# baresip/re

Hardware: AMD Instinct MI355X
Metric: GiB/s + Mpkt/s SRTP protect+unprotect, 1200B RTP pkts, device-resident (higher is better)
Workload: dtype u8

## Files before the change

re_amd/csrc/hip/k_ctr_fused.h:

```cpp
#pragma once
#include "k_ctr_fast.h"
#include "plan_common.h"

struct FArgs {
	KArgs a;
	struct sgpu_fused p;
};

#define FZ_BLOCK CTRF_BLOCK

struct FShared {
	uint32_t t;
	uint32_t fail;
	uint32_t hl0, ssrc0, seq0;
	uint32_t excl;
	uint32_t xfail;
	uint32_t wsum[FZ_BLOCK / 64];
	uint32_t seq[FZ_BLOCK + 2];
};

#ifdef FZ_WTIME
#define FZ_WTIME_MAX 4096u
#define FZ_WREC 24u
__device__ uint64_t g_fzw[FZ_WREC * FZ_WTIME_MAX];
#define FZ_STAMP(k)                                                          \
	do {                                                                 \
		if (threadIdx.x == 0 && S.t < FZ_WTIME_MAX)                  \
			g_fzw[FZ_WREC * S.t + 18u + (k)] =                   \
				__builtin_amdgcn_s_memrealtime();            \
	} while (0)
#else
#define FZ_STAMP(k) do { } while (0)
#endif

template <bool PROT>
__device__ __forceinline__ int fz_plan(const FArgs &fa, FShared &S,
				       uint8_t *smem, FastPkt &fp)
{
	const KArgs &a = fa.a;
	const struct sgpu_fused &P = fa.p;
	const struct sgpu_plan_in &in = P.in;
	const uint32_t tid = threadIdx.x, B = FZ_BLOCK;
	const uint32_t lane = tid & 63u, wv = tid >> 6;
	const uint64_t asz = a.asz;
	const uint32_t n = in.n;

	if (tid == 0) {
		S.t = atomicAdd(P.ticket, 1u) - P.tbase;
		S.fail = 0;
	}
	__syncthreads();
	FZ_STAMP(0);
	const uint32_t t = S.t;
	const uint32_t base = t * B, i = base + tid;
	const bool live = i < n;
	uint32_t p = 0, e = 0, cp = 0;
	struct sgpu_hdr h;
	h.ssrc = 0; h.seq = 0; h.err_pos = 0; h.hdr_len = 0xffffffffu;
	if (live) {
		p = P.pos[i];
		e = P.end[i];
		cp = P.cap ? P.cap[i] : 0u;
		const uint32_t left = (e > p && e <= asz) ? e - p : 0u;
		h = parse_rtp_hdr(a.arena + p, p, left);
	}
	if (tid < 3) {
		if (tid == 0) {
			const uint32_t q = P.pos[0], qe = P.end[0];
			const uint32_t left = (qe > q && qe <= asz) ? qe - q : 0u;
			const struct sgpu_hdr h0 = parse_rtp_hdr(a.arena + q, q,
								 left);
			S.hl0 = h0.hdr_len;
			S.ssrc0 = h0.ssrc;
			S.seq0 = h0.seq;
			if (t == 0) {
				P.out_next->fail = 0;
				P.out_next->nfail = 0;
				if (P.cm_out)
					*P.cm_out = P.comp;
			}
		}
		else if (base >= tid) {
			const uint32_t q = P.pos[base - tid];
			uint32_t sv = 0;
			if ((uint64_t)q + 4u <= asz)
				sv = (uint32_t)a.arena[q + 2] << 8 | a.arena[q + 3];
			S.seq[2 - tid] = sv;
		}
	}
#ifndef FZ_FILL_LOOP
	static_assert(FZ_BLOCK == 1024, "tt4_fill_b1024");
	tt4_fill_b1024(smem, a.t0);
#else
	tt4_fill(smem, a.t0);
#endif
	FZ_STAMP(4);
	if (live) {
		P.hdr[i] = h;
		P.es[i] = e;
		S.seq[tid + 2] = h.seq;
	}
	__syncthreads();
	FZ_STAMP(1);

	const uint32_t hl0 = S.hl0;
	const uint32_t ssrc0 = in.ssrc_any ? S.ssrc0 : in.ssrc;
	const uint32_t s_l0 = in.fresh ? S.seq0 : in.s_l;
	const uint32_t seq = h.seq;
	uint32_t f = 0, sb = 0;
	bool wrap = false;
	if (live) {
		sb = i == 0 ? s_l0 : S.seq[tid + 1];
		const uint32_t L = e - p;
		f |= plan_header_flags(h.hdr_len, hl0, h.ssrc, ssrc0,
				       PLAN_SSRC_PARSED, L, in.tag, 1, PROT);
		f |= plan_window_flags(p, e, P.cap != NULL, cp, asz, in.maxlen,
				       in.need, PROT);
		const struct plan_ord o = plan_order(seq, sb, i + 1 >= n, PROT);
		f |= o.flags;
		wrap = o.wrap;
		if (i == 0) {
			P.out->ssrc0 = h.ssrc;
			P.out->hl0 = h.hdr_len;
		}
	}
	if (tid == 0 && in.pred && *in.pred)
		f |= SPF_PRED;
	if (f)
		atomicOr(&S.fail, f);
	const uint64_t m = __ballot(wrap);
	if (lane == 0)
		S.wsum[wv] = (uint32_t)__popcll(m);
	__syncthreads();
	FZ_STAMP(2);

	if (wv == 0) {
		const uint32_t tot = wave_sum(lane < B / 64u ? S.wsum[lane] : 0u);
		const struct fz_prefix pf = fz_lookback(P.agg, P.epoch, t, lane,
							S.fail, tot,
							&P.out->fail);
		if (lane == 0) {
			S.excl = pf.excl;
			S.xfail = pf.fail;
		}
	}
	__syncthreads();
	FZ_STAMP(3);
	if (!live)
		return -1;
	if (S.xfail) {
		P.desc[i] = 0;
		return -1;
	}

	uint32_t pre = (uint32_t)__popcll(m & ((1ull << lane) - 1ull));
	for (uint32_t q = 0; q < wv; q++)
		pre += S.wsum[q];
	const uint32_t roc = in.roc + S.excl + pre + (wrap ? 1u : 0u);
	const struct plan_idx x = plan_index(roc, wrap, sb, seq, PROT);
	const uint64_t ix = x.ix;
	if (!PROT) {
		bool ok;
		if (i == 0) {
			ok = plan_new_first(ix, in.lix, in.bitmap);
		}
		else {
			const uint32_t psb = i == 1 ? s_l0 : S.seq[tid];
			ok = plan_new_later(ix, plan_prev_index(roc, wrap, psb, sb),
					    in.lix);
		}
		if (!ok)
			atomicOr(&P.out->fail, (uint32_t)SPF_REPLAY);
	}
	P.desc[i] = d_desc(ix, x.fl);
	const uint32_t t0 = n > SGPU_PLAN_TAIL ? n - SGPU_PLAN_TAIL : 0u;
	if (i >= t0)
		P.out->tail_ix[i - t0] = ix;
	if (i + 1 == n) {
		P.out->s_l_last = plan_s_l_after(seq, sb, wrap);
		P.out->wraps = roc - in.roc;
	}
	P.end[i] = e + (uint32_t)P.delta;
	P.err[i] = 0;
	fp.p = i;
	fp.off = p;
	fp.L = e - p;
	fp.hl = h.hdr_len;
	fp.ssrc = h.ssrc;
	fp.ixhi = (uint32_t)(ix >> 16);
	fp.ixlo = (uint32_t)(ix & 0xffffu);
	fp.roc = roc;
	return (int)((hl0 >> 2) & 3u);
}

template <int NR, bool PROT>
__global__ void
__attribute__((amdgpu_flat_work_group_size(1, FZ_BLOCK)))
__attribute__((amdgpu_waves_per_eu(FZ_BLOCK / 256, 8)))
k_ctr_fused(const FArgs fa)
{
#ifdef FZ_WTIME
	uint64_t t_start = 0;
	if (threadIdx.x == 0)
		t_start = __builtin_amdgcn_s_memrealtime();
#endif
	__shared__ __attribute__((aligned(16))) uint8_t smem[TT4_BYTES];
	__shared__ FShared S;
	FastPkt f;
	const int cls = fz_plan<PROT>(fa, S, smem, f);
#ifdef FZ_WTIME
	if (threadIdx.x == 0 && S.t < FZ_WTIME_MAX) {
		uint32_t hw;
		asm volatile("s_getreg_b32 %0, hwreg(HW_REG_HW_ID)" : "=s"(hw));
		g_fzw[FZ_WREC * S.t] = t_start;
		g_fzw[FZ_WREC * S.t + 1u] = hw;
	}
#endif
	if (cls < 0)
		return;
	const uint32_t ci = fa.p.comp;
	switch (cls) {
	case 0: ctr_fast_pkt<NR, 0, PROT>(fa.a, smem, f, ci); break;
	case 1: ctr_fast_pkt<NR, 1, PROT>(fa.a, smem, f, ci); break;
	case 2: ctr_fast_pkt<NR, 2, PROT>(fa.a, smem, f, ci); break;
	case 3: ctr_fast_pkt<NR, 3, PROT>(fa.a, smem, f, ci); break;
	default: break;
	}
#ifdef FZ_WTIME
	if ((threadIdx.x & 63u) == 0) {
		const uint32_t t = S.t;
		if (t < FZ_WTIME_MAX)
			g_fzw[FZ_WREC * t + 2u + threadIdx.x / 64u] =
				__builtin_amdgcn_s_memrealtime();
	}
#endif
}

#ifndef LP_PPT
#define LP_PPT 4
#endif
#define LP_WG (FZ_BLOCK * LP_PPT)

struct LpShared {
	uint32_t t, fail, hl0, ssrc0, seq0, excl, xfail;
	uint32_t wsum[LP_PPT][FZ_BLOCK / 64];
	uint32_t seq[LP_WG + 2];
};

template <bool PROT>
__global__ void __launch_bounds__(FZ_BLOCK)
k_lp_plan(const FArgs fa)
{
	__shared__ LpShared S;
	const KArgs &a = fa.a;
	const struct sgpu_fused &P = fa.p;
	const struct sgpu_plan_in &in = P.in;
	const uint32_t tid = threadIdx.x;
	const uint32_t lane = tid & 63u, wv = tid >> 6;
	const uint64_t asz = a.asz;
	const uint32_t n = in.n;

	if (tid == 0) {
		S.t = atomicAdd(P.ticket, 1u) - P.tbase;
		S.fail = 0;
	}
	__syncthreads();
	const uint32_t t = S.t;
	const uint32_t base = t * LP_WG;
	uint32_t pv[LP_PPT], ev[LP_PPT], cv[LP_PPT], w0[LP_PPT], w2[LP_PPT];
#pragma unroll
	for (int j = 0; j < LP_PPT; j++) {
		const uint32_t i = base + j * FZ_BLOCK + tid;
		pv[j] = ev[j] = cv[j] = 0;
		if (i < n) {
			pv[j] = P.pos[i];
			ev[j] = P.end[i];
			cv[j] = P.cap ? P.cap[i] : 0u;
		}
	}
#pragma unroll
	for (int j = 0; j < LP_PPT; j++) {
		const uint32_t p = pv[j], e = ev[j];
		w0[j] = w2[j] = 0;
		if (base + j * FZ_BLOCK + tid < n && e > p && e <= asz &&
		    e - p >= 12 && !(p & 3u)) {
			w0[j] = *(const uint32_t *)(a.arena + p);
			w2[j] = *(const uint32_t *)(a.arena + p + 8);
		}
	}
	if (tid < 3) {
		if (tid == 0) {
			const uint32_t q = P.pos[0], qe = P.end[0];
			const uint32_t left = (qe > q && qe <= asz) ? qe - q : 0u;
			const struct sgpu_hdr h0 = parse_rtp_hdr(a.arena + q, q,
								 left);
			S.hl0 = h0.hdr_len;
			S.ssrc0 = h0.ssrc;
			S.seq0 = h0.seq;
			if (t == 0) {
				P.out_next->fail = 0;
				P.out_next->nfail = 0;
				if (P.cm_out)
					*P.cm_out = P.comp;
				for (uint32_t c = 0; c < 4; c++)
					P.out->skip[c] =
						h0.hdr_len == 0xffffffffu ||
						((h0.hdr_len >> 2) & 3u) != c;
			}
		}
		else if (base >= tid) {
			const uint32_t q = P.pos[base - tid];
			uint32_t sv = 0;
			if ((uint64_t)q + 4u <= asz)
				sv = (uint32_t)a.arena[q + 2] << 8 | a.arena[q + 3];
			S.seq[2 - tid] = sv;
		}
	}
	struct sgpu_hdr hv[LP_PPT];
// ... 215 lines not shown
```

re_amd/csrc/hip/srtp_kernels.hip:

```cpp
#include <hip/hip_runtime.h>
#include <stddef.h>
#include <errno.h>
#include <stdio.h>
#include <string.h>
#include "../srtpgpu.h"
#include "kern_common.h"
#include "plan_common.h"
#include "k_ctr_fused.h"

#ifndef EAUTH
#define EAUTH 217
#endif


__device__ uint32_t g_T0[256];
__device__ uint8_t g_sbox[256];


__device__ uint8_t d_xt(uint8_t a) { return (uint8_t)((a << 1) ^ ((a & 0x80) ? 0x1b : 0)); }

__device__ void d_aes_expand(const uint8_t *key, uint32_t nk, uint8_t *rkb)
{
	uint32_t nr = nk + 6, i;
	uint8_t rcon = 1;
// ... 489 lines not shown
{
	const uint32_t left = (e > p && e <= asz) ? e - p : 0u;
	if (left < 12u + tag)
		return 0;
	const uint8_t *q = arena + e - 4u - tag;
	return (uint32_t)q[0] << 24 | (uint32_t)q[1] << 16 |
	       (uint32_t)q[2] << 8 | q[3];
}

__global__ void __launch_bounds__(PLAN_BLOCK)
k_rp_plan(const uint8_t *__restrict__ arena, uint64_t asz,
	  const struct sgpu_rfused R)
{
	__shared__ uint32_t ssrc0s, vw[PLAN_BLOCK + 1];
	const struct sgpu_rplan_in &in = R.in;
	const uint32_t tid = threadIdx.x;
	const uint32_t i = blockIdx.x * PLAN_BLOCK + tid;
	if (tid == 0) {
		const uint32_t q = R.pos[0], qe = R.end[0];
		const uint32_t left = (qe > q && qe <= asz) ? qe - q : 0u;
		ssrc0s = left >= 8 ? (uint32_t)arena[q + 4] << 24 |
				     (uint32_t)arena[q + 5] << 16 |
				     (uint32_t)arena[q + 6] << 8 | arena[q + 7]
				   : 0u;
		if (blockIdx.x == 0) {
			R.out_next->fail = 0;
			R.out_next->nfail = 0;
			if (R.cm_out)
				*R.cm_out = R.comp;
		}
		vw[0] = (!in.prot && i > 0 && i - 1 < in.n) ?
			rp_word(arena, asz, R.pos[i - 1], R.end[i - 1], in.tag)
			: 0u;
	}
	const bool live = i < in.n;
	uint32_t p = 0, e = 0, c = 0, v = 0;
	struct sgpu_hdr h;
	h.ssrc = 0; h.seq = 0; h.err_pos = 0; h.hdr_len = 0xffffffffu;
	if (live) {
		p = R.pos[i];
		e = R.end[i];
		c = R.cap ? R.cap[i] : 0u;
		const uint32_t left = (e > p && e <= asz) ? e - p : 0u;
		if (left >= 8) {
			const uint8_t *b = arena + p;
			h.ssrc = (uint32_t)b[4] << 24 | (uint32_t)b[5] << 16 |
				 (uint32_t)b[6] << 8 | b[7];
			h.hdr_len = 8;
		}
		if (!in.prot)
			v = rp_word(arena, asz, p, e, in.tag);
		R.hdr[i] = h;
		R.es[i] = e;
	}
	vw[tid + 1] = v;
	__syncthreads();
	if (!live)
		return;
	const uint32_t ssrc0 = in.ssrc_any ? ssrc0s : in.ssrc;
	const struct plan_rtcp r = plan_rtcp_packet(
		in, i, h.hdr_len != 0xffffffffu, h.ssrc, ssrc0, e - p,
		plan_window_flags(p, e, R.cap != NULL, c, asz, in.maxlen, in.need,
				  in.prot),
		v, vw[tid]);
	rplan_emit(r, i, in.n, h.ssrc, R.desc, R.out);
}


static char g_err[256];
static int g_inited;
static struct sgpu_session *g_table;
static struct sgpu_sstate *g_sst;
static uint32_t g_table_cap;
static struct sgpu_keyreq *g_req_dev;

extern "C" struct sgpu_sstate *sgpu_sst_table(void)
{
	return g_sst;
}
static uint32_t *g_slot_dev;
static uint32_t g_req_cap;

static const uint32_t *g_T0_dev;

static int herr(hipError_t e, const char *what)
{
	if (e == hipSuccess)
		return 0;
	snprintf(g_err, sizeof(g_err), "%s: %s", what, hipGetErrorString(e));
	return EIO;
}

extern "C" const char *sgpu_last_error(void) { return g_err; }

static uint8_t h_xt(uint8_t a) { return (uint8_t)((a << 1) ^ ((a & 0x80) ? 0x1b : 0)); }

extern "C" int sgpu_init(void)
{
	int n = 0;
	if (g_inited)
		return 0;
	if (hipGetDeviceCount(&n) != hipSuccess || n <= 0) {
		snprintf(g_err, sizeof(g_err), "no HIP device visible");
		return ENODEV;
	}
	uint8_t sbox[256];
	uint32_t T0[256];
	for (int x = 0; x < 256; x++) {
		uint8_t inv = 0;
		for (int y = 1; x && y < 256; y++) {
			uint8_t a = (uint8_t)x, b = (uint8_t)y, r = 0;
			while (b) {
				if (b & 1)
					r ^= a;
				a = h_xt(a);
				b >>= 1;
			}
			if (r == 1) {
				inv = (uint8_t)y;
				break;
			}
		}
		uint8_t s = inv;
		s = (uint8_t)(inv ^ (uint8_t)((inv << 1) | (inv >> 7)) ^
			      (uint8_t)((inv << 2) | (inv >> 6)) ^
			      (uint8_t)((inv << 3) | (inv >> 5)) ^
			      (uint8_t)((inv << 4) | (inv >> 4)) ^ 0x63);
		sbox[x] = s;
	}
	for (int x = 0; x < 256; x++) {
		uint8_t s = sbox[x], s2 = h_xt(s), s3 = (uint8_t)(s2 ^ s);
		T0[x] = (uint32_t)s2 | (uint32_t)s << 8 | (uint32_t)s << 16 |
			(uint32_t)s3 << 24;
	}
	int e = herr(hipMemcpyToSymbol(HIP_SYMBOL(g_sbox), sbox, 256), "sbox");
	if (!e)
		e = herr(hipMemcpyToSymbol(HIP_SYMBOL(g_T0), T0, 1024), "T0");
	if (!e)
		e = herr(hipGetSymbolAddress((void **)&g_T0_dev, HIP_SYMBOL(g_T0)),
			 "T0 address");
	if (e)
		return e;
	g_inited = 1;
	return 0;
}

extern "C" int sgpu_table_reserve(uint32_t nsessions)
{
	if (nsessions <= g_table_cap)
		return 0;
	uint32_t cap = g_table_cap ? g_table_cap : 1024;
	while (cap < nsessions)
		cap *= 2;
	struct sgpu_session *nt = NULL;
	struct sgpu_sstate *ns = NULL;
	int e = herr(hipMalloc(&nt, (size_t)cap * sizeof(*nt)), "table alloc");
	if (!e)
		e = herr(hipMalloc(&ns, (size_t)cap * sizeof(*ns)),
			 "state table alloc");
	if (e) {
		(void)hipFree(nt);
		return e;
	}
	if (g_table) {
		e = herr(hipMemcpy(nt, g_table,
				   (size_t)g_table_cap * sizeof(*nt),
				   hipMemcpyDeviceToDevice), "table grow");
		if (!e)
			e = herr(hipMemcpy(ns, g_sst,
					   (size_t)g_table_cap * sizeof(*ns),
					   hipMemcpyDeviceToDevice),
				 "state table grow");
		(void)hipDeviceSynchronize();
		(void)hipFree(g_table);
		(void)hipFree(g_sst);
	}
	g_table = nt;
	g_sst = ns;
	g_table_cap = cap;
	return e;
}


__global__ void k_gate_pred(const uint32_t *pred, uint32_t *fail)
{
	if (*pred)
		atomicOr(fail, (uint32_t)SPF_PRED);
}

__global__ void k_gate_set(const uint32_t *fail, const uint32_t *nfail,
			   uint32_t *gate)
{
	*gate = (*fail || (nfail && *nfail)) ? 1u : 0u;
}

extern "C" int sgpu_gate_pred(const uint32_t *pred, uint32_t *fail,
			      void *stream)
{
	hipLaunchKernelGGL(k_gate_pred, dim3(1), dim3(1), 0,
			   (hipStream_t)stream, pred, fail);
	return herr(hipGetLastError(), "k_gate_pred launch");
}

extern "C" int sgpu_gate_set(const uint32_t *fail, const uint32_t *nfail,
			     uint32_t *gate, void *stream)
{
	hipLaunchKernelGGL(k_gate_set, dim3(1), dim3(1), 0,
			   (hipStream_t)stream, fail, nfail, gate);
	return herr(hipGetLastError(), "k_gate_set launch");
}


__global__ void k_sst_zero(const uint32_t *slot, uint32_t n,
			   struct sgpu_sstate *sst)
{
	const uint32_t i = blockIdx.x * blockDim.x + threadIdx.x;
	if (i < n)
		sst[slot[i]] = sgpu_sstate{};
}

static_assert(sizeof(struct sgpu_sstate) == 32 &&
	      offsetof(struct sgpu_sstate, flags) == 12,
	      "sst_ld/sst_st move the state as two 16-byte words");

__device__ __forceinline__ void sst_ld(const struct sgpu_sstate *p, uint4 &a,
// ... 526 lines not shown
			      (hipStream_t)stream, sgpu_ctr_fast_mk_block(),
			      "k_ctr_fast_mk", nr, prot, 4);
		if (!e && !prot && c->flist) {
			const uint32_t g = c->n < 1024u ? c->n : 1024u;
			hipLaunchKernelGGL(nr == 10 ? sgpu_pick_ctr10_fast(0, 3)
						    : sgpu_pick_ctr14_fast(0, 3),
					   dim3(g), dim3(256), 0,
					   (hipStream_t)stream, a);
			e = herr(hipGetLastError(), "refix mk launch");
		}
		return e;
	}
	kfn_t f = mode == SGPU_MODE_GCM ?
			  sgpu_pick_gcm(true, c->uniform != 0, nr, prot)
		  : nr == 10 ? sgpu_pick_ctr10(true, c->uniform != 0, shift, prot)
			     : sgpu_pick_ctr14(true, c->uniform != 0, shift, prot);
	if (!f) {
		snprintf(g_err, sizeof(g_err), "no kernel for mode %d nr %d",
			 mode, nr);
		return EINVAL;
	}
	KArgs a;
	memset(&a, 0, sizeof(a));
	a.arena = arena;
	a.asz = arena_size;
	a.comps = (const struct sgpu_comp *)g_table;
	a.t0 = g_T0_dev;
	a.verdict = c->verdict;
	a.save = c->save;
	a.c = *c;
	return launch(f, a, c->n,
		      c->undo ? -1 : prof_slot(mode, nr, shift < 0 ? 3 : shift,
					       prot),
		      (hipStream_t)stream,
		      mode == SGPU_MODE_GCM ? sgpu_gcm_block(c->uniform != 0)
					    : sgpu_ctr_block(c->uniform != 0, prot),
		      mode == SGPU_MODE_GCM ?
			      (c->uniform ? "k_gcmu" : "k_gcm_compact") :
		      shift < 0 ? (c->uniform ? "k_ctr_hmac_any_uni"
					      : "k_ctr_hmac_any") :
				  (c->uniform ? "k_ctr_hmac_uni"
					      : "k_ctr_hmac_compact"),
		      nr, prot, mode == SGPU_MODE_CTR && shift < 0 ? 4 : 1);
}


static void fz_args(FArgs &fa, uint8_t *arena, uint64_t asz,
		   const struct sgpu_fused *f)
{
	memset(&fa, 0, sizeof(fa));
	KArgs &a = fa.a;
	a.arena = arena;
	a.asz = asz;
	a.comps = (const struct sgpu_comp *)g_table;
	a.t0 = g_T0_dev;
	a.verdict = f->verdict;
	a.save = f->save;
	a.c.pos = f->pos;
	a.c.end = f->es;
	a.c.hdr = f->hdr;
	a.c.desc = f->desc;
	a.c.compmap = f->cm_out;
	a.c.n = f->in.n;
	a.c.verdict = f->verdict;
	a.c.save = f->save;
	a.c.nfail = &f->out->nfail;
	a.c.flist = f->flist;
	a.c.uniform = 2;
	fa.p = *f;
}

extern "C" unsigned sgpu_fused_block(void)
{
	return FZ_BLOCK;
}

extern "C" int sgpu_run_fused(uint8_t *arena, uint64_t arena_size,
			      struct sgpu_fused *f, int nr, void *stream)
{
	FArgs fa;
	if (!f->in.n || (nr != 10 && nr != 14))
		return EINVAL;
	const int prot = f->in.prot != 0;
	const uint32_t nwg = (f->in.n + FZ_BLOCK - 1) / FZ_BLOCK;
	f->ntickets = nwg;
	fz_args(fa, arena, arena_size, f);
	return launch_fused(sgpu_pick_fused(nr, prot, 0), fa, nwg * FZ_BLOCK,
			    f->in.n, prof_slot(SGPU_MODE_CTR, nr, 3, prot),
			    (hipStream_t)stream, FZ_BLOCK, "k_ctr_fused", nr,
			    prot, &f->prof_id);
}

extern "C" int sgpu_run_fzplan(uint8_t *arena, uint64_t arena_size,
			       struct sgpu_fused *f, void *stream)
{
	FArgs fa;
	if (!f->in.n)
		return EINVAL;
	const uint32_t wg = sgpu_lp_wg();
	const uint32_t nwg = (f->in.n + wg - 1) / wg;
	f->ntickets = nwg;
	f->prof_id = 0;
	fz_args(fa, arena, arena_size, f);
	hipLaunchKernelGGL(sgpu_pick_fzplan(f->in.prot != 0), dim3(nwg),
			   dim3(FZ_BLOCK), 0, (hipStream_t)stream, fa);
	return herr(hipGetLastError(), "plan launch");
}

extern "C" int sgpu_fused_undo(uint8_t *arena, uint64_t arena_size,
			       const struct sgpu_fused *f, int nr, int prot,
			       void *stream)
{
	FArgs fa;
	if (!f->in.n || (nr != 10 && nr != 14) || f->shift > 3)
		return EINVAL;
	fz_args(fa, arena, arena_size, f);
	hipLaunchKernelGGL(sgpu_pick_fused(nr, prot, 1),
			   dim3((f->in.n + FZ_BLOCK - 1) / FZ_BLOCK),
			   dim3(FZ_BLOCK), 0, (hipStream_t)stream, fa);
	return herr(hipGetLastError(), "fused undo launch");
}

extern "C" int sgpu_fused_refix(uint8_t *arena, uint64_t arena_size,
				const struct sgpu_fused *f, int nr,
				void *stream)
{
	FArgs fa;
	if (!f->in.n || (nr != 10 && nr != 14))
		return EINVAL;
	fz_args(fa, arena, arena_size, f);
	const uint32_t g = f->in.n < 1024u ? f->in.n : 1024u;
	hipLaunchKernelGGL(nr == 10 ? sgpu_pick_ctr10_fast(0, 2)
				    : sgpu_pick_ctr14_fast(0, 2),
			   dim3(g), dim3(256), 0, (hipStream_t)stream, fa.a);
	return herr(hipGetLastError(), "fused refix launch");
}

extern "C" int sgpu_parse_headers(const uint8_t *arena, uint64_t arena_size,
				  const uint32_t *pos, const uint32_t *end,
				  struct sgpu_hdr *out, uint32_t *eix, uint32_t n,
				  int rtcp, void *stream)
{
	if (!n)
		return 0;
	struct sgpu_prologue pro;
	memset(&pro, 0, sizeof(pro));
	return sgpu_parse_prologue(arena, arena_size, pos, end, out, eix, n,
				   rtcp, &pro, stream);
}

extern "C" int sgpu_parse_prologue(const uint8_t *arena, uint64_t arena_size,
				   const uint32_t *pos, const uint32_t *end,
				   struct sgpu_hdr *out, uint32_t *eix,
				   uint32_t n, int rtcp,
				   const struct sgpu_prologue *pro,
				   void *stream)
{
	if (!n)
		return 0;
	hipLaunchKernelGGL(k_parse, dim3((n + 255) / 256), dim3(256), 0,
			   (hipStream_t)stream, arena, arena_size, pos, end, out,
			   eix, n, rtcp, *pro);
	return herr(hipGetLastError(), "k_parse launch");
}

__global__ void k_rx_pack(const struct sgpu_hdr *__restrict__ hd,
			  const int32_t *__restrict__ res, uint32_t ssrc0,
			  uint32_t *__restrict__ out, uint32_t n)
// ... 604 lines not shown
```

re_amd/csrc/host/batch_dev.c:

```c
#include <errno.h>
#include <pthread.h>
#include <stdatomic.h>
#include <stdio.h>
#include <stdlib.h>
#include <string.h>
#include <time.h>
#include "re_mem.h"
#include "re_mbuf.h"
#include "re_srtp.h"
#include "re_srtp_batch.h"
#include "re_rtcp_batch.h"
#include "../srtpgpu.h"
#include "../hip/plan_rx_rule.h"
#include "bp_layout.h"
#include "fault.h"
#include "pool.h"
#include "srtp_int.h"


static struct sgpu_compact compact_of(const struct srtp_batch_dev *d,
				      const struct ws_layout *L)
{
	return (struct sgpu_compact){
		.pos = d->pos, .end = L->es, .hdr = L->hdr, .desc = L->desc,
// ... 269 lines not shown
}

static int plan_out_back(struct dcall *k, struct sgpu_plan_out *out,
			 void *host, void *stream)
{
	const int sync = k->sync;
	int err = 0;
	k->devfold = 0;
	if (!g_env.nopost) {
		uint32_t *done = NULL;
		if (sync && g_env.syncspin && sync_word(k->w))
			done = k->w->sy_word;
		k->spin = done ? ++k->w->sy_seq : 0;
		if (k->spin == 0 && done)
			k->spin = ++k->w->sy_seq;
		return sgpu_plan_post(out, host, sizeof(*out),
				      sync ? NULL : k->gate, done, k->spin,
				      stream);
	}
	if (!sync && k->gate)
		err = sgpu_plan_finish(&out->fail, NULL, NULL, NULL, 0, 0,
				       &out->nfail, k->gate, NULL, NULL, stream);
	if (!err)
		err = sgpu_memcpy_d2h(host, out, sizeof(*out), stream);
	return err;
}

static int fz_issue(struct dcall *k)
{
	const int prot = k->op == OP_RTP_ENC;
	struct srtp *s = k->sessv[0];
	struct srtp_batch_dev *d = &k->d;
	const struct comp *c0 = &s->rtp;
	const int gcm = c0->mode == SGPU_MODE_GCM;
	const size_t n = d->n;
	const uint32_t T = gcm ? 16u : c0->tag_len;
	const uint32_t need = prot ? (gcm ? 16u : (T > 4 ? T : 4u)) : 0u;
	const uint32_t B = sgpu_fused_block();
	const uint32_t nblk = (uint32_t)((n + B - 1) / B);
	const struct ws_sizes z = {
		.hd = n * sizeof(struct sgpu_hdr), .dsc = n * 8,
		.vs = n * 9 + 72, .cm = 4, .pl = 64 + (n / 256 + 4) * 20,
		.es = n * 4, .es_first = 1};
	struct ws *w = k->w;
	struct sgpu_fused *F = &k->fz;
	struct ws_layout L;
	struct fz_layout Z;
	void *stream = d->stream;
	int err;

	err = ws_layout_reserve(w, n, &z, &L);
	if (!err)
		err = fz_prepare(w, nblk, stream);
	if (err)
		return err;
	k->foff = w->fz_par;
	Z = fz_layout_get(w, w->fz_par);

	memset(F, 0, sizeof(*F));
	plan_in(&F->in, s, (uint32_t)n, prot, T, need);
	F->in.zeroed = 1;
	F->in.pred = k->pred;
	F->pos = d->pos;
	F->end = d->end;
	F->cap = d->cap;
	F->err = d->err;
	F->es = L.es;
	F->hdr = L.hdr;
	F->desc = L.desc;
	if (!prot) {
		F->save = L.save;
		F->verdict = L.verdict;
		F->flist = gcm ? NULL : L.flist;
	}
	F->out = Z.out;
	F->out_next = Z.out_next;
	F->cm_out = L.cm;
	F->agg = Z.agg;
	F->ticket = Z.ticket;
	F->tbase = w->fz_tbase;
	F->epoch = w->fz_epoch;
	F->comp = c0->dev;
	F->delta = prot ? (int32_t)T : -(int32_t)T;
	err = k->fused == 1 ? sgpu_run_fused(d->arena, d->arena_size, F,
					     (int)c0->nr, stream)
			    : sgpu_run_fzplan(d->arena, d->arena_size, F, stream);
	if (err) {
		w->fz_d = NULL;
		return err;
	}
	w->fz_tbase += F->ntickets;
	w->fz_epoch++;
	w->fz_par ^= 1;
	if (k->fused == 2) {
		struct sgpu_compact C = {
			.pos = d->pos, .end = F->es, .hdr = F->hdr,
			.desc = F->desc, .compmap = F->cm_out, .n = (uint32_t)n,
			.verdict = F->verdict, .save = F->save,
			.nfail = &F->out->nfail, .uniform = gcm ? 1 : 2,
			.guard = gcm ? &F->out->fail : F->out->skip,
			.flist = F->flist, .gfail = gcm ? NULL : &F->out->fail};
		err = sgpu_run_compact(d->arena, d->arena_size, &C, c0->mode,
				       (int)c0->nr, gcm ? 0 : -1, prot, stream);
		if (err)
			return err;
	}
	return plan_out_back(k, F->out, Z.out_h, stream);
}

static int fz_finish(struct dcall *k)
{
	const int prot = k->op == OP_RTP_ENC;
	const int lean = k->fused == 2;
	struct srtp *s = k->sessv[0];
	struct srtp_batch_dev *d = &k->d;
	const struct comp *c0 = &s->rtp;
	const int gcm = c0->mode == SGPU_MODE_GCM;
	const size_t n = d->n;
	const unsigned ns0 = s->nstreams;
	struct ws *w = k->w;
	struct sgpu_fused *F = &k->fz;
	const struct fz_layout Z = fz_layout_get(w, (uint32_t)k->foff);
	const struct sgpu_plan_out *po = Z.out_h;
	void *stream = d->stream;
	struct srtp_stream old;
	int err = 0;

	k->pfail = po->fail;
	if (po->fail) {
		if (!lean)
			sgpu_prof_void(F->prof_id);
		if (plan_rejected(po->fail, ns0) == -2)
			return -2;
		if (po->fail & (SPF_BAD | SPF_SLOW))
			w->fz_d = NULL;
		if (po->fail & SPF_SLOW)
			count(&g_cnt_lbtimeout, 1);
		if (!lean)
			goto undo;
		if (g_env.times)
			fprintf(stderr, "re_srtp plan n=%zu %s: rejected "
				"(SPF %#x)\n", n, prot ? "protect" : "unprotect",
				po->fail);
		return undone(0, d, F->es);
	}
	plan_apply(s, po, prot, n, &old);
	count(lean ? &g_cnt_lplans : &g_cnt_fused, 1);
	if (!po->nfail)
		return 0;
	count(&g_cnt_misses, po->nfail);
	if (!g_env.nodevfold) {
		if (!gcm)
			err = sgpu_fused_refix(d->arena, d->arena_size, F,
					       (int)c0->nr, stream);
		if (!err)
			err = sgpu_fold_rtp(0, &F->out->nfail, &F->in, F->hdr,
					    F->desc, F->verdict, F->es, d->pos,
					    d->end, d->err, gcm,
					    (uint32_t *)(w->pl.d + 64), Z.fo,
					    stream);
		if (!err)
			err = sgpu_memcpy_d2h(Z.fo_h, Z.fo, sizeof(*Z.fo),
					      stream);
		if (!err)
			err = sgpu_stream_sync(stream);
		if (err)
// ... 1967 lines not shown
```

re_amd/csrc/host/srtp.c:

```c
#include <errno.h>
#include <pthread.h>
#include <stdatomic.h>
#include <stdio.h>
#include <stdlib.h>
#include <string.h>
#include <time.h>
#include "re_mem.h"
#include "re_mbuf.h"
#include "re_srtp.h"
#include "re_srtp_batch.h"
#include "re_rtcp_batch.h"
#include "../srtpgpu.h"
#include "fault.h"
#include "pool.h"
#include "srtp_int.h"



__thread struct tk_owner *t_own;

struct tk_owner *tk_me(void)
{
	if (!t_own)
		t_own = fi_calloc(1, sizeof(*t_own));
// ... 134 lines not shown
	if (!strcmp(name, "pcpackets"))
		return __atomic_load_n(&g_cnt_pcpkts, __ATOMIC_RELAXED);
	if (!strcmp(name, "rxw_redos"))
		return __atomic_load_n(&g_cnt_rxw_redo, __ATOMIC_RELAXED);
	if (!strcmp(name, "pcfused"))
		return __atomic_load_n(&g_cnt_pcfused, __ATOMIC_RELAXED);
	if (!strcmp(name, "gated"))
		return __atomic_load_n(&g_cnt_gated, __ATOMIC_RELAXED);
	if (!strcmp(name, "small_launches"))
		return __atomic_load_n(&g_cnt_small, __ATOMIC_RELAXED);
	if (!strcmp(name, "small_ns_launch"))
		return __atomic_load_n(&g_ns_small_launch, __ATOMIC_RELAXED);
	if (!strcmp(name, "small_ns_sync"))
		return __atomic_load_n(&g_ns_small_sync, __ATOMIC_RELAXED);
	if (!strcmp(name, "fused_ns_prep"))
		return __atomic_load_n(&g_ns_fused_prep, __ATOMIC_RELAXED);
	if (!strcmp(name, "fused_ns_post"))
		return __atomic_load_n(&g_ns_fused_post, __ATOMIC_RELAXED);
	if (!strcmp(name, "sync_calls"))
		return __atomic_load_n(&g_cnt_sync_calls, __ATOMIC_RELAXED);
	if (!strcmp(name, "sync_ns_issue"))
		return __atomic_load_n(&g_ns_sync_issue, __ATOMIC_RELAXED);
	if (!strcmp(name, "sync_ns_wait"))
		return __atomic_load_n(&g_ns_sync_wait, __ATOMIC_RELAXED);
	if (!strcmp(name, "sync_ns_finish"))
		return __atomic_load_n(&g_ns_sync_finish, __ATOMIC_RELAXED);
	if (!strcmp(name, "mbufs_ns"))
		return __atomic_load_n(&g_ns_mbufs, __ATOMIC_RELAXED);
	if (!strcmp(name, "freshmulti"))
		return (uint64_t)__atomic_load_n(&g_fresh_multi, __ATOMIC_RELAXED);
	if (!strcmp(name, "prof_voided"))
		return sgpu_prof_voided();
	if (!strcmp(name, "fail_alloc"))
		return (uint64_t)__atomic_load_n(&re_amd_fail_alloc,
						 __ATOMIC_RELAXED);
	if (!strcmp(name, "mem_live"))
		return re_amd_mem_live ? re_amd_mem_live() : 0;
	if (!strcmp(name, "slots_live"))
		return slots_live();
	return 0;
}

int srtp_gpu_tune(const char *name, long value)
{
	env_init();
	if (!name)
		return EINVAL;
	if (!strcmp(name, "noplan"))
		g_env.noplan = value > 0;
	else if (!strcmp(name, "general"))
		g_env.general = value > 0;
	else if (!strcmp(name, "perclass"))
		g_env.perclass = value > 0;
	else if (!strcmp(name, "nolean"))
		g_env.nolean = value > 0;
	else if (!strcmp(name, "nodevfold"))
		g_env.nodevfold = value > 0;
	else if (!strcmp(name, "splan"))
		g_env.splan = value > 0;
	else if (!strcmp(name, "nomk"))
		g_env.nomk = value > 0;
	else if (!strcmp(name, "nobucket"))
		g_env.nobucket = value > 0;
	else if (!strcmp(name, "mpradix"))
		g_env.mpradix = value > 0;
	else if (!strcmp(name, "nocoop"))
		sgpu_set_coop(value <= 0);
	else if (!strcmp(name, "nocombine"))
		g_env.nocombine = value > 0;
	else if (!strcmp(name, "nosmall"))
		g_env.nosmall = value > 0;
	else if (!strcmp(name, "lplan"))
		g_env.lplan = value > 0;
	else if (!strcmp(name, "nopost"))
		g_env.nopost = value > 0;
	else if (!strcmp(name, "bpexp"))
		sgpu_bplan_set_exp(value > 0 && value <= SGPU_BP_CAPMAX ?
				   (uint32_t)value : 0u);
	else if (!strcmp(name, "noplanfuse"))
		g_env.noplanfuse = value > 0;
	else if (!strcmp(name, "fzepoch"))
		__atomic_store_n(&g_env.fzepoch, value > 0 ? value : 0,
				 __ATOMIC_RELAXED);
	else if (!strcmp(name, "nofuse"))
		g_env.nofuse = value > 0;
	else if (!strcmp(name, "smallsync"))
		g_env.smallsync = value > 0;
	else if (!strcmp(name, "norxplan"))
		g_env.norxplan = value > 0;
	else if (!strcmp(name, "nomrplan"))
		g_env.nomrplan = value > 0;
	else if (!strcmp(name, "nomrrxplan"))
		g_env.nomrrxplan = value > 0;
	else if (!strcmp(name, "nomsplan"))
		g_env.nomsplan = value > 0;
	else if (!strcmp(name, "nomsrxplan"))
		g_env.nomsrxplan = value > 0;
	else if (!strcmp(name, "nosrxplan"))
		g_env.nosrxplan = value > 0;
	else if (!strcmp(name, "nosrplan"))
		g_env.nosrplan = value > 0;
	else if (!strcmp(name, "rxseq"))
		g_env.rxseq = value > 0;
	else if (!strcmp(name, "freshmulti"))
		__atomic_store_n(&g_fresh_multi, value > 0, __ATOMIC_RELAXED);
	else if (!strcmp(name, "pcrunners"))
		g_env.pcrunners = value > 0 ? value : 0;
	else if (!strcmp(name, "pchold"))
		g_env.pchold = value > 0 ? value : 0;
	else if (!strcmp(name, "syncspin"))
		g_env.syncspin = value > 0;
	else if (!strcmp(name, "pclinger"))
		g_env.pclinger = value > 0 ? (value < 10000 ? value : 10000) : 0;
	else if (!strcmp(name, "pcspin"))
		g_env.pcspin = value > 0 ? value : 0;
	else if (!strcmp(name, "trace"))
		g_env.trace = value > 0;
	else if (!strcmp(name, "times"))
		g_env.times = value > 0;
	else if (!strcmp(name, "chunk"))
		g_env.chunk = value >= 64 ? (size_t)value : (size_t)1 << 18;
	else if (!strcmp(name, "par_min"))
		g_env.par_min = value > 0 ? (size_t)value : 4096;
	else if (!strcmp(name, "fail_grow"))
		__atomic_store_n(&g_fail_grow, value > 0 ? value : 0,
				 __ATOMIC_RELAXED);
	else if (!strcmp(name, "fail_alloc"))
		__atomic_store_n(&re_amd_fail_alloc, value > 0 ? value : 0,
				 __ATOMIC_RELAXED);
	else
		return EINVAL;
	return 0;
}


static pthread_mutex_t g_lock = PTHREAD_MUTEX_INITIALIZER;
static pthread_rwlock_t g_table_rw = PTHREAD_RWLOCK_INITIALIZER;
static uint32_t *g_free;
static uint32_t g_nfree, g_free_cap, g_next_slot;
static int g_gpu_state;

int gpu_ready(void)
{
	int r;
	pthread_mutex_lock(&g_lock);
	if (g_gpu_state == 0) {
		int e = sgpu_init();
		g_gpu_state = e ? -1 : 1;
		if (e)
			fprintf(stderr, "re_srtp_amd: no HIP device usable "
				"(%s); srtp_alloc returns ENOSYS\n",
				sgpu_last_error());
	}
	r = g_gpu_state;
	pthread_mutex_unlock(&g_lock);
	return r == 1;
}

const char *srtp_gpu_error(void)
{
	return sgpu_last_error();
}

static int slots_get(uint32_t *slots, size_t n)
{
	size_t i;
// ... 1579 lines not shown
```

re_amd/csrc/host/srtp_int.h:

```cpp
#ifndef RE_AMD_SRTP_INT_H
#define RE_AMD_SRTP_INT_H

#include <errno.h>
#include <pthread.h>
#include <stdint.h>
#include <stdlib.h>
#include <string.h>
#include <time.h>
#include "re_mem.h"
#include "re_mbuf.h"
#include "re_srtp.h"
#include "re_srtp_batch.h"
#include "../srtpgpu.h"
#include "fault.h"
#include "pool.h"

#ifndef EAUTH
#define EAUTH 217
#endif

#define SRTP_MAX_STREAMS 8

enum { OP_RTP_ENC = 0, OP_RTP_DEC = 1, OP_RTCP_ENC = 2, OP_RTCP_DEC = 3 };

struct replay {
	uint64_t bitmap;
	uint64_t lix;
};

struct srtp_stream {
	struct replay replay_rtp;
	struct replay replay_rtcp;
	uint32_t ssrc;
	uint32_t roc;
	uint16_t s_l;
	uint8_t s_l_set;
	uint32_t rtcp_index;
	uint32_t epoch;
};

struct comp {
	int has_aes;
	int mode;
	int has_hmac;
	int encrypted;
	uint32_t tag_len;
	uint32_t nr;
	uint32_t dev;
};

struct srtp {
	unsigned nstreams;
	uint32_t slot;
	int suite;
	struct srtp_stream streams[SRTP_MAX_STREAMS];
	struct comp rtp, rtcp;
	int dev;
	uint32_t mp_epoch;
	int dres;
	uint64_t pend_p;
	uint64_t pend_m;
	const struct tk_owner *pend_own;
};

struct tk_owner {
	uint64_t done;
};

struct srtp_env {
	int noplan;
	int general;
	int perclass;
	int nolean;
	int nocombine;
	int nomk;
	int splan;
	int nobucket;
	int mpradix;
	int nodevfold;
	int nosmall;
	long pcrunners;
	long pchold;
	int syncspin;
	long pclinger;
	long pcspin;
	int rxseq;
	int norxplan;
	int nomsplan;
	int nomsrxplan;
	int nosrxplan;
	int nosrplan;
	int nomrplan;
	int nomrrxplan;
	int smallsync;
	int lplan;
	int nopost;
	int noplanfuse;
	long fzepoch;
	int nofuse;
	int trace;
	int times;
	size_t chunk;
	size_t par_min;
};
extern struct srtp_env g_env;

struct pinfo {
	uint32_t start, end, size;
	uint32_t hdr_len;
	uint32_t err_pos;
	uint32_t ssrc;
	uint16_t seq;
	uint32_t eix[3];
	uint8_t fixed;
};

struct rec {
	int32_t err;
	uint32_t pos_o, end_o, size_o;
	uint8_t has_job;
	uint8_t need_run;
	uint8_t ran;
	uint8_t vd;
	uint8_t need_undo;
	uint32_t in_end;
	uint32_t ext_end;
	struct sgpu_job job;
	struct sgpu_job ran_job;
	uint32_t save;
};

struct engine {
	int op;
	size_t n;
	struct srtp **sess;
	struct pinfo *pi;
	struct rec *rec;
	struct srtp **uniq;
	size_t nuniq;
	struct srtp *snap;
};

struct pool {
	uint8_t *h;
	uint8_t *d;
	size_t cap;
};

struct ulog {
	struct srtp *s;
	struct srtp_stream *st;
	unsigned nstreams;
	struct srtp_stream old;
};

struct ulogv {
	struct ulog *v;
	size_t n, cap;
};

struct ws {
	void *stream;
	struct pool ctl;
	struct pool stage;
	struct pool hdr;
	uint32_t *cls_idx;
	size_t cls_cap;
	void *pstream;
	struct pool up;
	struct pool hd;
	struct pool dsc;
	struct pool vs;
	struct pool cm;
	struct pool pl;
	struct pool es;
	struct pool ms;
	struct pool mscr;
	void **ev;
	void *upev;
	size_t nev;
	struct ulogv ulog[1];
// ... 266 lines not shown
```

re_amd/csrc/srtpgpu.h:

```cpp
#ifndef SRTPGPU_H
#define SRTPGPU_H

#include <stdint.h>
#include <stddef.h>

#ifdef __cplusplus
extern "C" {
#endif

enum {
	SGPU_MODE_CTR = 0,
	SGPU_MODE_GCM = 1,
};

struct sgpu_comp {
	uint32_t rk[60];
	uint32_t nr;
	uint32_t mode;
	uint32_t tag_len;
	uint32_t flags;
	uint32_t k_s[4];
	uint32_t ipad[5];
	uint32_t opad[5];
	uint32_t pad0[2];
// ... 134 lines not shown


int   sgpu_run_compact(uint8_t *arena, uint64_t arena_size,
		       const struct sgpu_compact *c, int mode, int nr,
		       int shift, int prot, void *stream);

struct sgpu_plan_in {
	uint32_t n;
	uint32_t prot;
	uint32_t fresh;
	uint32_t ssrc;
	uint32_t roc;
	uint32_t s_l;
	uint64_t lix;
	uint64_t bitmap;
	uint32_t tag;
	uint32_t ssrc_any;
	uint32_t need;
	uint32_t maxlen;
	uint32_t zeroed;
	uint32_t pad;
	const uint32_t *pred;
};

#define SGPU_CACHED_MAX_CTR (4096u - 64u)
#define SGPU_CACHED_MAX_GCM (4096u - 64u)
#define SGPU_CACHED_MAX(mode) \
	((mode) == SGPU_MODE_GCM ? SGPU_CACHED_MAX_GCM : SGPU_CACHED_MAX_CTR)

enum {
	SPF_PARSE   = 1u << 0,
	SPF_SSRC    = 1u << 1,
	SPF_CLASS   = 1u << 2,
	SPF_ORDER   = 1u << 3,
	SPF_TIMEOUT = 1u << 4,
	SPF_REPLAY  = 1u << 5,
	SPF_SIZE    = 1u << 6,
	SPF_CAP     = 1u << 7,
	SPF_BAD     = 1u << 8,
	SPF_PRED    = 1u << 9,
	SPF_SEG     = 1u << 10,
	SPF_SLOW    = 1u << 11,
};
#define SGPU_MP_SEGMAX 1024

int   sgpu_gate_pred(const uint32_t *pred, uint32_t *fail, void *stream);
int   sgpu_gate_set(const uint32_t *fail, const uint32_t *nfail,
		    uint32_t *gate, void *stream);

#define SGPU_PLAN_TAIL 65
struct sgpu_plan_out {
	uint32_t fail;
	uint32_t wraps;
	uint32_t ssrc0;
	uint32_t hl0;
	uint32_t s_l_last;
	uint32_t nfail;
	uint32_t skip[4];
	uint64_t tail_ix[SGPU_PLAN_TAIL];
};

struct sgpu_fused {
	struct sgpu_plan_in in;
	const uint32_t *pos;
	uint32_t *end;
	const uint32_t *cap;
	int32_t *err;
	uint32_t *es;
	struct sgpu_hdr *hdr;
	uint64_t *desc;
	uint8_t *verdict;
	uint32_t *save;
	uint32_t *flist;
	struct sgpu_plan_out *out;
	struct sgpu_plan_out *out_next;
	uint32_t *cm_out;
	unsigned long long *agg;
	uint32_t *ticket;
	uint32_t tbase;
	uint32_t epoch;
	uint32_t comp;
	int32_t delta;
	uint32_t shift;
	uint32_t ntickets;
	uint64_t prof_id;
};
unsigned sgpu_fused_block(void);
int   sgpu_run_fzplan(uint8_t *arena, uint64_t arena_size,
		      struct sgpu_fused *f, void *stream);
int   sgpu_run_fused(uint8_t *arena, uint64_t arena_size,
		     struct sgpu_fused *f, int nr, void *stream);
int   sgpu_fused_undo(uint8_t *arena, uint64_t arena_size,
		      const struct sgpu_fused *f, int nr, int prot,
		      void *stream);
int   sgpu_fused_refix(uint8_t *arena, uint64_t arena_size,
		       const struct sgpu_fused *f, int nr, void *stream);

int   sgpu_plan_rtp(const struct sgpu_plan_in *in, const struct sgpu_hdr *hdr,
		    const uint32_t *pos, const uint32_t *end, const uint32_t *cap,
		    uint64_t arena_size, uint64_t *desc, uint32_t *scratch,
		    struct sgpu_plan_out *out, void *stream);

struct sgpu_rxplan_in {
	uint32_t n;
	uint32_t fresh;
	uint32_t ssrc;
	uint32_t ssrc_any;
	uint32_t roc;
	uint32_t s_l;
	uint64_t lix;
	uint64_t bitmap;
	uint32_t tag;
	uint32_t maxlen;
	uint32_t hmac;
	uint32_t lookback;
	uint32_t zeroed;
	uint32_t pad;
};

struct sgpu_rxplan_out {
	uint32_t fail;
	uint32_t nfail;
	uint32_t roc;
	uint32_t s_l;
	uint64_t lix;
	uint64_t bitmap;
	uint32_t nlate;
	uint32_t ndup;
	uint32_t skip[4];
	uint32_t ssrc0;
	uint32_t hl0;
};

size_t sgpu_plan_rx_scratch(uint32_t n);
int   sgpu_plan_rx(const struct sgpu_rxplan_in *in, const struct sgpu_hdr *hdr,
		   const uint32_t *pos, const uint32_t *end, const uint32_t *cap,
		   uint64_t arena_size, uint64_t *desc, void *scratch,
		   size_t scratch_bytes, struct sgpu_rxplan_out *out,
		   void *stream);
int   sgpu_plan_rx_commit(const struct sgpu_rxplan_out *out,
			  const struct sgpu_hdr *hdr, const void *scratch,
			  const uint32_t *es, uint32_t *pos, uint32_t *end,
			  int32_t *err, uint32_t n, uint32_t tag, void *stream);

enum {
	SST_EXISTS  = 1u << 0,
	SST_SL_SET  = 1u << 1,
	SST_TOUCHED = 1u << 2,
};

struct sgpu_sstate {
	uint32_t ssrc;
	uint32_t roc;
	uint32_t s_l;
	uint32_t flags;
	uint64_t lix;
	uint64_t bitmap;
};

#define SGPU_SP_MAX 8
struct sgpu_splan_in {
	uint32_t n;
	uint32_t prot;
	uint32_t tag;
	uint32_t need;
	uint32_t maxlen;
// ... 446 lines not shown
```

Baseline: 506.2.

## Make fused CTR kernel persistent with wave-level planning of next tile

Launches the fused plan+CTR kernel with a grid sized to the number of compute units (or a tunable fzgrid) and loops over tickets. The first wave to finish encryption plans the next tile into shared-memory records while the other waves are still encrypting. This hides the plan phase's latency behind cipher work and cuts the cost of launching and scheduling many workgroups. In exchange it adds spin-waits on shared counters, more LDS per block (which may lower occupancy), serialises the whole plan onto one wave, and changes the ticket accounting.

```diff
diff --git a/re_amd/csrc/hip/k_ctr_fused.h b/re_amd/csrc/hip/k_ctr_fused.h
--- a/re_amd/csrc/hip/k_ctr_fused.h
+++ b/re_amd/csrc/hip/k_ctr_fused.h
@@ -8,6 +8,9 @@
 };
 
 #define FZ_BLOCK CTRF_BLOCK
+#define FZ_NONE 0xffffffffu
+#define FZ_LATE (-2)
+#define FZ_RECW 6
 
 struct FShared {
 	uint32_t t;
@@ -17,6 +20,13 @@
 	uint32_t xfail;
 	uint32_t wsum[FZ_BLOCK / 64];
 	uint32_t seq[FZ_BLOCK + 2];
+	uint32_t nxt;
+	uint32_t home;
+	uint32_t rd;
+	uint32_t rec[FZ_RECW][FZ_BLOCK];
+#ifdef FZ_WTIME
+	uint32_t wt[FZ_BLOCK / 64];
+#endif
 };
 
 #ifdef FZ_WTIME
@@ -48,10 +58,15 @@
 	if (tid == 0) {
 		S.t = atomicAdd(P.ticket, 1u) - P.tbase;
 		S.fail = 0;
-	}
-	__syncthreads();
+		S.nxt = S.t;
+		S.home = 0;
+		S.rd = 0;
+	}
+	__syncthreads();
+	const uint32_t t = S.t;
+	if (t >= (n + B - 1u) / B)
+		return FZ_LATE;
 	FZ_STAMP(0);
-	const uint32_t t = S.t;
 	const uint32_t base = t * B, i = base + tid;
 	const bool live = i < n;
 	uint32_t p = 0, e = 0, cp = 0;
@@ -193,6 +208,197 @@
 	return (int)((hl0 >> 2) & 3u);
 }
 
+__device__ __forceinline__ void fz_park(FShared &S, const FastPkt &fp, int cls)
+{
+	const uint32_t tid = threadIdx.x;
+	S.rec[0][tid] = fp.off;
+	S.rec[1][tid] = fp.L;
+	S.rec[2][tid] = fp.hl;
+	S.rec[3][tid] = fp.ixhi;
+	S.rec[4][tid] = cls < 0 ? 0u : fp.ixlo | (uint32_t)(cls + 1) << 16;
+	S.rec[5][tid] = fp.roc;
+}
+
+__device__ __forceinline__ void fz_wave_sync(void)
+{
+	__builtin_amdgcn_fence(__ATOMIC_RELEASE, "wavefront");
+	__builtin_amdgcn_wave_barrier();
+	__builtin_amdgcn_fence(__ATOMIC_ACQUIRE, "wavefront");
+}
+
+__device__ __forceinline__ const FArgs &fz_args_again(void)
+{
+	auto p = __builtin_amdgcn_kernarg_segment_ptr();
+	asm volatile("" : "+s"(p));
+	return *(const FArgs *)p;
+}
+
+#define FZ_PPL (FZ_BLOCK / 64)
+#define FZ_PG 4
+
+template <bool PROT>
+__device__ __forceinline__ void fz_plan_next(FShared &S)
+{
+	const FArgs &fa = fz_args_again();
+	const KArgs &a = fa.a;
+	const struct sgpu_fused &P = fa.p;
+	const struct sgpu_plan_in &in = P.in;
+	const uint32_t lane = threadIdx.x & 63u, B = FZ_BLOCK;
+	const uint64_t asz = a.asz;
+	const uint32_t n = in.n;
+
+	uint32_t t = 0;
+	if (lane == 0)
+		t = atomicAdd(P.ticket, 1u) - P.tbase;
+	t = __builtin_amdgcn_readfirstlane(t);
+	while (__hip_atomic_load(&S.rd, __ATOMIC_RELAXED,
+				 __HIP_MEMORY_SCOPE_WORKGROUP) != B / 64u)
+		__builtin_amdgcn_s_sleep(1);
+	__builtin_amdgcn_fence(__ATOMIC_ACQUIRE, "workgroup");
+	if (lane == 0)
+		__hip_atomic_store(&S.rd, 0u, __ATOMIC_RELAXED,
+				   __HIP_MEMORY_SCOPE_WORKGROUP);
+	if (t >= (n + B - 1u) / B) {
+		if (lane == 0)
+			S.nxt = FZ_NONE;
+		return;
+	}
+	const uint32_t base = t * B;
+	if (lane - 1u < 2u) {
+		const uint32_t q = P.pos[base - lane];
+		uint32_t sv = 0;
+		if ((uint64_t)q + 4u <= asz)
+			sv = (uint32_t)a.arena[q + 2] << 8 | a.arena[q + 3];
+		S.seq[2 - lane] = sv;
+	}
+	const uint32_t hl0 = S.hl0;
+	const uint32_t ssrc0 = in.ssrc_any ? S.ssrc0 : in.ssrc;
+	uint32_t f = 0;
+#pragma unroll 1
+	for (uint32_t g = 0; g < FZ_PPL; g += FZ_PG) {
+		uint32_t pv[FZ_PG], ev[FZ_PG], cv[FZ_PG], w0[FZ_PG], w2[FZ_PG];
+#pragma unroll
+		for (int j = 0; j < FZ_PG; j++) {
+			const uint32_t i = base + (g + j) * 64u + lane;
+			pv[j] = ev[j] = cv[j] = 0;
+			if (i < n) {
+				pv[j] = P.pos[i];
+				ev[j] = P.end[i];
+				cv[j] = P.cap ? P.cap[i] : 0u;
+			}
+		}
+#pragma unroll
+		for (int j = 0; j < FZ_PG; j++) {
+			const uint32_t p = pv[j], e = ev[j];
+			w0[j] = w2[j] = 0;
+			if (base + (g + j) * 64u + lane < n && e > p && e <= asz &&
+			    e - p >= 12 && !(p & 3u)) {
+				w0[j] = *(const uint32_t *)(a.arena + p);
+				w2[j] = *(const uint32_t *)(a.arena + p + 8);
+			}
+		}
+#pragma unroll
+		for (int j = 0; j < FZ_PG; j++) {
+			const uint32_t q = (g + j) * 64u + lane, i = base + q;
+			if (i >= n)
+				continue;
+			const uint32_t p = pv[j], e = ev[j];
+			const uint32_t left = (e > p && e <= asz) ? e - p : 0u;
+			struct sgpu_hdr h;
+			if (left >= 12 && !(p & 3u) && !(w0[j] & 0x1fu)) {
+				h.seq = (uint16_t)((w0[j] >> 8 & 0xff00u) |
+						   (w0[j] >> 24));
+				h.ssrc = __builtin_bswap32(w2[j]);
+				h.err_pos = 0;
+				h.hdr_len = 12;
+			}
+			else {
+				h = parse_rtp_hdr(a.arena + p, p, left);
+			}
+			P.hdr[i] = h;
+			P.es[i] = e;
+			S.seq[q + 2] = h.seq;
+			S.rec[0][q] = p;
+			S.rec[1][q] = e - p;
+			S.rec[2][q] = h.hdr_len;
+			f |= plan_header_flags(h.hdr_len, hl0, h.ssrc, ssrc0,
+					       PLAN_SSRC_PARSED, e - p, in.tag, 1,
+					       PROT);
+			f |= plan_window_flags(p, e, P.cap != NULL, cv[j], asz,
+					       in.maxlen, in.need, PROT);
+		}
+	}
+	fz_wave_sync();
+
+	uint32_t wm = 0, tot = 0;
+#pragma unroll 1
+	for (uint32_t j = 0; j < FZ_PPL; j++) {
+		const uint32_t q = j * 64u + lane, i = base + q;
+		bool wrap = false;
+		if (i < n) {
+			const struct plan_ord o = plan_order(S.seq[q + 2],
+							     S.seq[q + 1],
+							     i + 1 >= n, PROT);
+			f |= o.flags;
+			wrap = o.wrap;
+		}
+		tot += (uint32_t)__popcll(__ballot(wrap));
+		wm |= (wrap ? 1u : 0u) << j;
+	}
+	if (lane == 0 && in.pred && *in.pred)
+		f |= SPF_PRED;
+	const struct fz_prefix pf = fz_lookback(P.agg, P.epoch, t, lane,
+						wave_or(f), tot, &P.out->fail);
+	const bool dead = pf.fail != 0;
+
+	const uint32_t cls1 = ((hl0 >> 2) & 3u) + 1u;
+	const uint32_t t0 = n > SGPU_PLAN_TAIL ? n - SGPU_PLAN_TAIL : 0u;
+	uint32_t pre = in.roc + pf.excl;
+#pragma unroll 1
+	for (uint32_t j = 0; j < FZ_PPL; j++) {
+		const uint32_t q = j * 64u + lane, i = base + q;
+		const bool wrap = (wm >> j) & 1u;
+		const uint64_t m = __ballot(wrap);
+		const uint32_t roc = pre +
+			(uint32_t)__popcll(m & ((1ull << lane) - 1ull)) +
+			(wrap ? 1u : 0u);
+		pre += (uint32_t)__popcll(m);
+		uint32_t w4 = 0;
+		if (i < n && dead) {
+			P.desc[i] = 0;
+		}
+		else if (i < n) {
+			const uint32_t seq = S.seq[q + 2], sb = S.seq[q + 1];
+			const struct plan_idx x = plan_index(roc, wrap, sb, seq,
+							     PROT);
+			const uint64_t ix = x.ix;
+			if (!PROT) {
+				if (!plan_new_later(ix,
+						    plan_prev_index(roc, wrap,
+								    S.seq[q], sb),
+						    in.lix))
+					atomicOr(&P.out->fail,
+						 (uint32_t)SPF_REPLAY);
+			}
+			P.desc[i] = d_desc(ix, x.fl);
+			if (i >= t0)
+				P.out->tail_ix[i - t0] = ix;
+			if (i + 1 == n) {
+				P.out->s_l_last = plan_s_l_after(seq, sb, wrap);
+				P.out->wraps = roc - in.roc;
+			}
+			P.end[i] = S.rec[0][q] + S.rec[1][q] + (uint32_t)P.delta;
+			P.err[i] = 0;
+			S.rec[3][q] = (uint32_t)(ix >> 16);
+			S.rec[5][q] = roc;
+			w4 = (uint32_t)(ix & 0xffffu) | cls1 << 16;
+		}
+		S.rec[4][q] = w4;
+	}
+	if (lane == 0)
+		S.nxt = t;
+}
+
 template <int NR, bool PROT>
 __global__ void
 __attribute__((amdgpu_flat_work_group_size(1, FZ_BLOCK)))
@@ -206,34 +412,76 @@
 #endif
 	__shared__ __attribute__((aligned(16))) uint8_t smem[TT4_BYTES];
 	__shared__ FShared S;
-	FastPkt f;
-	const int cls = fz_plan<PROT>(fa, S, smem, f);
+	{
+		FastPkt f;
+		const int cls = fz_plan<PROT>(fa, S, smem, f);
+		if (cls == FZ_LATE)
+			return;
+		fz_park(S, f, cls);
+	}
 #ifdef FZ_WTIME
-	if (threadIdx.x == 0 && S.t < FZ_WTIME_MAX) {
-		uint32_t hw;
-		asm volatile("s_getreg_b32 %0, hwreg(HW_REG_HW_ID)" : "=s"(hw));
+	if (threadIdx.x == 0 && S.t < FZ_WTIME_MAX)
 		g_fzw[FZ_WREC * S.t] = t_start;
-		g_fzw[FZ_WREC * S.t + 1u] = hw;
-	}
 #endif
-	if (cls < 0)
-		return;
-	const uint32_t ci = fa.p.comp;
-	switch (cls) {
-	case 0: ctr_fast_pkt<NR, 0, PROT>(fa.a, smem, f, ci); break;
-	case 1: ctr_fast_pkt<NR, 1, PROT>(fa.a, smem, f, ci); break;
-	case 2: ctr_fast_pkt<NR, 2, PROT>(fa.a, smem, f, ci); break;
-	case 3: ctr_fast_pkt<NR, 3, PROT>(fa.a, smem, f, ci); break;
-	default: break;
-	}
+	for (;;) {
+		__syncthreads();
+		const uint32_t tid = threadIdx.x;
+		if (S.nxt == FZ_NONE)
+			break;
+		const FArgs &fb = fz_args_again();
+		FastPkt f;
+		f.off = S.rec[0][tid];
+		f.L = S.rec[1][tid];
+		f.hl = S.rec[2][tid];
+		f.ixhi = S.rec[3][tid];
+		const uint32_t w4 = S.rec[4][tid];
+		f.roc = S.rec[5][tid];
+		f.ixlo = w4 & 0xffffu;
+		f.p = S.nxt * FZ_BLOCK + tid;
+		f.ssrc = fb.p.in.ssrc_any ? S.ssrc0 : fb.p.in.ssrc;
 #ifdef FZ_WTIME
-	if ((threadIdx.x & 63u) == 0) {
-		const uint32_t t = S.t;
-		if (t < FZ_WTIME_MAX)
-			g_fzw[FZ_WREC * t + 2u + threadIdx.x / 64u] =
-				__builtin_amdgcn_s_memrealtime();
-	}
+		if ((tid & 63u) == 0)
+			S.wt[tid / 64u] = S.nxt;
+		if (tid == 0 && S.nxt < FZ_WTIME_MAX) {
+			const uint64_t now = __builtin_amdgcn_s_memrealtime();
+			uint32_t hw;
+			asm volatile("s_getreg_b32 %0, hwreg(HW_REG_HW_ID)" : "=s"(hw));
+			if (S.nxt != S.t) {
+				g_fzw[FZ_WREC * S.nxt] = now;
+				for (uint32_t k = 18; k < 23; k++)
+					g_fzw[FZ_WREC * S.nxt + k] = now;
+			}
+			g_fzw[FZ_WREC * S.nxt + 1u] = hw;
+		}
 #endif
+		__builtin_amdgcn_fence(__ATOMIC_RELEASE, "workgroup");
+		if ((tid & 63u) == 0)
+			atomicAdd(&S.rd, 1u);
+		const uint32_t ci = fb.p.comp;
+		switch ((int)(w4 >> 16) - 1) {
+		case 0: ctr_fast_pkt<NR, 0, PROT>(fb.a, smem, f, ci); break;
+		case 1: ctr_fast_pkt<NR, 1, PROT>(fb.a, smem, f, ci); break;
+		case 2: ctr_fast_pkt<NR, 2, PROT>(fb.a, smem, f, ci); break;
+		case 3: ctr_fast_pkt<NR, 3, PROT>(fb.a, smem, f, ci); break;
+		default: break;
+		}
+#ifdef FZ_WTIME
+		if ((threadIdx.x & 63u) == 0) {
+			const uint32_t t = S.wt[threadIdx.x / 64u];
+			if (t < FZ_WTIME_MAX)
+				g_fzw[FZ_WREC * t + 2u + threadIdx.x / 64u] =
+					__builtin_amdgcn_s_memrealtime();
+		}
+#endif
+		uint32_t h = 0;
+		if ((threadIdx.x & 63u) == 0)
+			h = atomicAdd(&S.home, 1u);
+		h = __builtin_amdgcn_readfirstlane(h);
+		if (h == FZ_BLOCK / 64u - 1u && (threadIdx.x & 63u) == 0)
+			S.home = 0;
+		if (h == 0)
+			fz_plan_next<PROT>(S);
+	}
 }
 
 #ifndef LP_PPT
diff --git a/re_amd/csrc/hip/srtp_kernels.hip b/re_amd/csrc/hip/srtp_kernels.hip
--- a/re_amd/csrc/hip/srtp_kernels.hip
+++ b/re_amd/csrc/hip/srtp_kernels.hip
@@ -595,6 +595,7 @@
 static uint32_t g_req_cap;
 
 static const uint32_t *g_T0_dev;
+static uint32_t g_ncu;
 
 static int herr(hipError_t e, const char *what)
 {
@@ -654,6 +655,12 @@
 			 "T0 address");
 	if (e)
 		return e;
+	int dev = 0, ncu = 0;
+	if (hipGetDevice(&dev) != hipSuccess ||
+	    hipDeviceGetAttribute(&ncu, hipDeviceAttributeMultiprocessorCount,
+				  dev) != hipSuccess || ncu <= 0)
+		return herr(hipErrorInvalidDevice, "compute unit count");
+	g_ncu = (uint32_t)ncu;
 	g_inited = 1;
 	return 0;
 }
@@ -1346,8 +1353,10 @@
 	if (!f->in.n || (nr != 10 && nr != 14))
 		return EINVAL;
 	const int prot = f->in.prot != 0;
-	const uint32_t nwg = (f->in.n + FZ_BLOCK - 1) / FZ_BLOCK;
-	f->ntickets = nwg;
+	const uint32_t nt = (f->in.n + FZ_BLOCK - 1) / FZ_BLOCK;
+	const uint32_t want = f->grid ? f->grid : g_ncu;
+	const uint32_t nwg = want < nt ? want : nt;
+	f->ntickets = nt + nwg;
 	fz_args(fa, arena, arena_size, f);
 	return launch_fused(sgpu_pick_fused(nr, prot, 0), fa, nwg * FZ_BLOCK,
 			    f->in.n, prof_slot(SGPU_MODE_CTR, nr, 3, prot),
diff --git a/re_amd/csrc/host/batch_dev.c b/re_amd/csrc/host/batch_dev.c
--- a/re_amd/csrc/host/batch_dev.c
+++ b/re_amd/csrc/host/batch_dev.c
@@ -375,6 +375,7 @@
 	F->epoch = w->fz_epoch;
 	F->comp = c0->dev;
 	F->delta = prot ? (int32_t)T : -(int32_t)T;
+	F->grid = g_env.fzgrid;
 	err = k->fused == 1 ? sgpu_run_fused(d->arena, d->arena_size, F,
 					     (int)c0->nr, stream)
 			    : sgpu_run_fzplan(d->arena, d->arena_size, F, stream);
diff --git a/re_amd/csrc/host/srtp.c b/re_amd/csrc/host/srtp.c
--- a/re_amd/csrc/host/srtp.c
+++ b/re_amd/csrc/host/srtp.c
@@ -240,6 +240,8 @@
 	else if (!strcmp(name, "fzepoch"))
 		__atomic_store_n(&g_env.fzepoch, value > 0 ? value : 0,
 				 __ATOMIC_RELAXED);
+	else if (!strcmp(name, "fzgrid"))
+		g_env.fzgrid = value > 0 && value <= 0xffff ? (uint32_t)value : 0u;
 	else if (!strcmp(name, "nofuse"))
 		g_env.nofuse = value > 0;
 	else if (!strcmp(name, "smallsync"))
diff --git a/re_amd/csrc/host/srtp_int.h b/re_amd/csrc/host/srtp_int.h
--- a/re_amd/csrc/host/srtp_int.h
+++ b/re_amd/csrc/host/srtp_int.h
@@ -97,6 +97,7 @@
 	int nopost;
 	int noplanfuse;
 	long fzepoch;
+	uint32_t fzgrid;
 	int nofuse;
 	int trace;
 	int times;
diff --git a/re_amd/csrc/srtpgpu.h b/re_amd/csrc/srtpgpu.h
--- a/re_amd/csrc/srtpgpu.h
+++ b/re_amd/csrc/srtpgpu.h
@@ -240,6 +240,7 @@
 	uint32_t comp;
 	int32_t delta;
 	uint32_t shift;
+	uint32_t grid;
 	uint32_t ntickets;
 	uint64_t prof_id;
 };
```

Result: no change. 507.8 (median of 6 runs) (+0.3%).
